# dmMaze/comic-text-detector

Hardware: AMD Instinct MI355X
Metric: pages/sec at 1024x1024 bs=32 (end-to-end detector, device-resident pages) (higher is better)
Workload: dtype f16

## Files before the change

### comic-text-detector_amd/csrc/kernels_twlds.hip

```cpp
#include <algorithm>

#include "kernels.h"
#include "tail.h"

namespace {

constexpr int TL_MAXT = 1024;

struct Geo {
  int W, H, wp, words;
  unsigned last;
};

__device__ __forceinline__ unsigned lds_ld(const unsigned* p) {
  return __hip_atomic_load(p, __ATOMIC_RELAXED, __HIP_MEMORY_SCOPE_WORKGROUP);
}
__device__ __forceinline__ void lds_st(unsigned* p, unsigned v) {
  __hip_atomic_store(p, v, __ATOMIC_RELAXED, __HIP_MEMORY_SCOPE_WORKGROUP);
}

struct Row3 {
  unsigned prev, cur, nxt;
};
__device__ __forceinline__ Row3 row3(const unsigned* p, const Geo& g, int y, int wi) {
  Row3 r{0u, 0u, 0u};
  if ((unsigned)y < (unsigned)g.H) {
    const unsigned* q = p + y * g.wp + wi;
    r.cur = q[0];
    if (wi > 0) r.prev = q[-1];
    if (wi + 1 < g.wp) r.nxt = q[1];
  }
  return r;
}
template <int K> __device__ __forceinline__ unsigned shk(const Row3& r) {
  if constexpr (K == 0) return r.cur;
  else if constexpr (K > 0) return (r.cur >> K) | (r.nxt << (32 - K));
  else return (r.cur << -K) | (r.prev >> (32 + K));
}
__device__ __forceinline__ unsigned ring3(const Row3& r) { return shk<-1>(r) | r.cur | shk<1>(r); }

__device__ __forceinline__ unsigned upto(int p) { return ~(~1u << p); }

__device__ __forceinline__ void load32(const uint8_t* p, int n, unsigned* v) {
  if (n >= 32) {
    __builtin_memcpy(v, p, 16);
    __builtin_memcpy(v + 4, p + 16, 16);
    return;
  }
#pragma unroll
  for (int j = 0; j < 8; ++j) {
    unsigned x = 0;
    if (4 * j + 4 <= n) {
      __builtin_memcpy(&x, p + 4 * j, 4);
    } else {
      for (int k = 0; k < 3; ++k)
        if (4 * j + k < n) x |= (unsigned)p[4 * j + k] << (8 * k);
    }
    v[j] = x;
  }
}

__device__ __forceinline__ unsigned gt60_nibble(unsigned x) {
  const unsigned t = (((x & 0x7f7f7f7fu) + 0x43434343u) | x) & 0x80808080u;
  const unsigned g = t >> 7;
  return (g | (g >> 7) | (g >> 14) | (g >> 21)) & 0xfu;
}

__device__ __forceinline__ int gray3(unsigned b, unsigned g, unsigned r) {
  return (int)((b * 3735u + g * 19235u + r * 9798u + 16384u) >> 15);
}

__device__ __forceinline__ unsigned uf_find(unsigned* parent, unsigned a) {
  for (;;) {
    const unsigned p = lds_ld(parent + a);
    if (p == a) return a;
    const unsigned gp = lds_ld(parent + p);
    if (gp != p) lds_st(parent + a, gp);
    a = gp;
  }
}
__device__ __forceinline__ void uf_union(unsigned* parent, unsigned a, unsigned b) {
  for (;;) {
    a = uf_find(parent, a);
    b = uf_find(parent, b);
    if (a == b) return;
    if (a < b) {
      const unsigned t = a;
      a = b;
      b = t;
    }
    if (atomicCAS(parent + a, a, b) == a) return;
  }
}

struct TLdsArgs {
  const TWin* wins;
  const TBand* bands;
  const int* order;
  int dilate;
  int max_words, rlay;
  int rcap;
  int* ovf;
};

__global__ __launch_bounds__(TL_MAXT) void tw_lds_kernel(TLdsArgs a) {
  extern __shared__ __attribute__((aligned(16))) unsigned lds[];
  const int t = threadIdx.x, lane = t & 63, wave = t >> 6;
  const int TL_NT = blockDim.x, NWV = TL_NT >> 6;
  const int widx = a.order[blockIdx.x];
  const TWin w = a.wins[widx];
  Geo g;
  g.W = w.w, g.H = w.h, g.wp = (w.w + 31) >> 5, g.words = g.wp * g.H;
  g.last = (w.w & 31) ? ((1u << (w.w & 31)) - 1u) : 0xffffffffu;
  const int MW = a.max_words, RL = a.rlay, RC = a.rcap;
  unsigned* const pred = lds;
  unsigned* const merged = lds + MW;
  unsigned* const cand = lds + 2 * MW;
  unsigned short* const base = (unsigned short*)(lds + 3 * MW);
  unsigned* const parent = lds + 3 * MW + ((MW + 1) >> 1);
  int* const acc = (int*)(parent + RL);
  unsigned* const red = parent + 2 * RL;
  unsigned* const tmp = parent;
  auto validw = [&](int wi) { return wi == g.wp - 1 ? g.last : 0xffffffffu; };
  const int y_t = t / g.wp, wi_t = t - y_t * g.wp;
  const int dy_t = TL_NT / g.wp, dwi_t = TL_NT - dy_t * g.wp;
  auto for_words = [&](auto&& fn) {
    int y = y_t, wi = wi_t;
    for (int i = t; i < g.words; i += TL_NT) {
      fn(i, y, wi);
      wi += dwi_t, y += dy_t;
      if (wi >= g.wp) wi -= g.wp, ++y;
    }
  };

  for_words([&](int i, int y, int wi) {
    unsigned v[8];
    load32(w.mask + (size_t)(w.y1 + y) * w.mask_w + w.x1 + 32 * wi, g.W - 32 * wi, v);
    unsigned bits = 0;
#pragma unroll
    for (int j = 0; j < 8; ++j) bits |= gt60_nibble(v[j]) << (4 * j);
    tmp[i] = bits & validw(wi);
    merged[i] = 0;
  });
  __syncthreads();
  for_words([&](int i, int y, int wi) {
    auto ext = [&](int yy, int ww) -> unsigned {
      if ((unsigned)yy >= (unsigned)g.H || (unsigned)ww >= (unsigned)g.wp) return 0xffffffffu;
      return tmp[yy * g.wp + ww] | ~validw(ww);
    };
    const unsigned cur = ext(y, wi), prev = ext(y, wi - 1), nxt = ext(y, wi + 1);
    pred[i] = cur & ((cur << 1) | (prev >> 31)) & ((cur >> 1) | (nxt << 31)) & ext(y - 1, wi) & ext(y + 1, wi) & validw(wi);
  });
  __syncthreads();

  const int seg = (g.words + TL_NT - 1) / TL_NT;
  auto starts_of = [&](int i, int wi) -> unsigned {
    const unsigned c = cand[i], cl = wi > 0 ? cand[i - 1] : 0u;
    return c & ~((c << 1) | (cl >> 31));
  };
  auto scan_runs = [&]() -> int {
    const int i0 = min(t * seg, g.words), i1 = min(i0 + seg, g.words);
    int cnt = 0;
    {
      int wi = i0 % g.wp;
      for (int i = i0; i < i1; ++i) {
        cnt += __popc(starts_of(i, wi));
        if (++wi == g.wp) wi = 0;
      }
    }
    int inc = cnt;
#pragma unroll
    for (int off = 1; off < 64; off <<= 1) {
      const int v = __shfl_up(inc, off);
      if (lane >= off) inc += v;
    }
    if (lane == 63) red[wave] = (unsigned)inc;
    __syncthreads();
    int before = inc - cnt;
    int total = 0;
    for (int k = 0; k < NWV; ++k) {
      const int v = (int)red[k];
      before += k < wave ? v : 0;
      total += v;
    }
    {
      int wi = i0 % g.wp, run = before;
      for (int i = i0; i < i1; ++i) {
        base[i] = (unsigned short)run;
        const int n = __popc(starts_of(i, wi));
        for (int k = run; k < run + n && k < RL; ++k) parent[k] = (unsigned)k, acc[k] = 0;
        run += n;
        if (++wi == g.wp) wi = 0;
      }
    }
    __syncthreads();
    return total;
  };
  auto rid_from = [](unsigned b, unsigned s, int p) -> unsigned { return b + (unsigned)__popc(s & upto(p)) - 1u; };
  auto for_groups = [&](unsigned v, auto&& fn) {
    while (v) {
      const unsigned lb = v & (0u - v);
      const unsigned grp = v & ~(v + lb);
      fn(__ffs((int)v) - 1, grp);
      v &= ~grp;
    }
  };
  auto link_and = [&](auto&& fn) {
    for_words([&](int i, int y, int wi) {
      const unsigned c = cand[i];
      if (!c) return;
      const unsigned cl = wi > 0 ? cand[i - 1] : 0u;
      const unsigned sc = c & ~((c << 1) | (cl >> 31)), bc = base[i];
      unsigned up = 0, ul = 0, ur = 0, su = 0, bu = 0;
      if (y > 0) {
        up = cand[i - g.wp];
        if (wi > 0) ul = cand[i - g.wp - 1];
        if (wi + 1 < g.wp) ur = cand[i - g.wp + 1];
        su = up & ~((up << 1) | (ul >> 31));
        bu = base[i - g.wp];
      }
      for_groups(c, [&](int p, unsigned grp) {
        const unsigned me = rid_from(bc, sc, p);
        fn(i, grp, me);
        if (y == 0) return;
        const unsigned an = up & (grp | (grp << 1) | (grp >> 1));
        unsigned reps = an & ~(an << 1);
        while (reps) {
          const int q = __ffs((int)reps) - 1;
          reps &= reps - 1;
          uf_union(parent, me, rid_from(bu, su, q));
        }
        if ((grp & 1u) && (ul >> 31)) uf_union(parent, me, bu - 1u);
        if ((grp >> 31) && (ur & 1u)) uf_union(parent, me, (unsigned)base[i - g.wp + 1] + ((up >> 31) ? 0u : 1u) - 1u);
      });
    });
  };
  auto fold_to_roots = [&](int n) {
    for (int i = t; i < n; i += TL_NT) {
      const unsigned r = uf_find(parent, (unsigned)i);
      if (r != (unsigned)i) {
        const int v = acc[i];
        if (v) atomicAdd(acc + r, v);
      }
    }
    __syncthreads();
  };
  auto or_accepted = [&]() {
    for_words([&](int i, int, int wi) {
      const unsigned c = cand[i];
      if (!c) return;
      const unsigned cl = wi > 0 ? cand[i - 1] : 0u;
      const unsigned sc = c & ~((c << 1) | (cl >> 31)), bc = base[i];
      unsigned add = 0;
      for_groups(c, [&](int p, unsigned grp) {
        if (acc[uf_find(parent, rid_from(bc, sc, p))] > 0) add |= grp;
      });
      if (add) merged[i] |= add;
    });
    __syncthreads();
  };
  bool overflow = false;

  for (int r = 0; r < w.nband && !overflow; ++r) {
    const TBand bd = a.bands[w.band0 + r];
    for_words([&](int i, int y, int wi) {
      const int npx = min(32, g.W - 32 * wi);
      const uint8_t* src = w.img + ((size_t)(w.y1 + y) * w.img_w + w.x1 + 32 * wi) * 3;
      unsigned v[24];
      load32(src, min(32, 3 * npx), v);
      load32(src + 32, min(32, max(0, 3 * npx - 32)), v + 8);
      load32(src + 64, min(32, max(0, 3 * npx - 64)), v + 16);
      unsigned bits = 0;
      auto byte_at = [&](int o) { return (v[o >> 2] >> (8 * (o & 3))) & 0xffu; };
      if (bd.kind == 0) {
#pragma unroll
        for (int k = 0; k < 32; ++k) {
          const int gr = gray3(byte_at(3 * k), byte_at(3 * k + 1), byte_at(3 * k + 2));
          bits |= ((gr >= bd.lo && gr <= bd.hi) ? 1u : 0u) << k;
        }
      } else {
        const int ch = bd.kind - 1;
#pragma unroll
        for (int k = 0; k < 32; ++k) {
          const unsigned c0 = byte_at(3 * k), c1 = byte_at(3 * k + 1), c2 = byte_at(3 * k + 2);
          bits |= (((int)(ch == 0 ? c0 : (ch == 1 ? c1 : c2)) > bd.lo) ? 1u : 0u) << k;
        }
      }
      if (bd.invert) bits = ~bits;
      tmp[i] = bits & validw(wi);
    });
    __syncthreads();
    for_words([&](int i, int y, int wi) {
      const Row3 c0 = row3(tmp, g, y, wi);
      unsigned out = c0.cur;
      if (out) {
        const Row3 m1 = row3(tmp, g, y - 1, wi), p1 = row3(tmp, g, y + 1, wi), m2 = row3(tmp, g, y - 2, wi), p2 = row3(tmp, g, y + 2, wi);
        const unsigned up = ring3(m1), dn = ring3(p1), cur = c0.cur;
        const unsigned single = cur & ~(shk<-1>(c0) | shk<1>(c0) | up | dn);
        const unsigned hl = cur & shk<1>(c0) & ~(shk<-1>(c0) | shk<2>(c0) | up | dn | shk<2>(m1) | shk<2>(p1));
        const unsigned hr = cur & shk<-1>(c0) & ~(shk<-2>(c0) | shk<1>(c0) | up | dn | shk<-2>(m1) | shk<-2>(p1));
        const unsigned vt = cur & p1.cur & ~(shk<-1>(c0) | shk<1>(c0) | shk<-1>(p1) | shk<1>(p1) | up | ring3(p2));
        const unsigned vb = cur & m1.cur & ~(shk<-1>(c0) | shk<1>(c0) | shk<-1>(m1) | shk<1>(m1) | dn | ring3(m2));
        out = cur & ~(single | hl | hr | vt | vb);
      }
      cand[i] = out;
    });
    __syncthreads();
    const int nr = scan_runs();
    if (nr > RC) {
      overflow = true;
      break;
    }
    link_and([&](int i, unsigned grp, unsigned me) {
      const unsigned nm = grp & ~merged[i];
      const int wgt = __popc(nm & pred[i]) - __popc(nm & ~pred[i]);
      if (wgt) atomicAdd(acc + me, wgt);
    });
    __syncthreads();
    fold_to_roots(nr);
    or_accepted();
  }

  if (!overflow) {
    if (a.dilate) {
      for_words([&](int i, int y, int wi) {
        unsigned v = 0;
#pragma unroll
        for (int dy = -1; dy <= 1; ++dy) {
          const Row3 r = row3(merged, g, y + dy, wi);
          v |= ring3(r);
        }
        tmp[i] = v & validw(wi);
      });
      __syncthreads();
    }
    unsigned cnt = 0;
    for_words([&](int i, int, int wi) {
      const unsigned m = a.dilate ? tmp[i] : merged[i];
      merged[i] = m;
      cand[i] = ~m & validw(wi);
      cnt += (unsigned)__popc(m);
    });
    for (int off = 32; off > 0; off >>= 1) cnt += __shfl_down(cnt, off);
    __syncthreads();
    if (lane == 0) red[wave] = cnt;
    if (t == 0) red[16] = 0u, red[17] = 0u, red[18] = 0u;
    __syncthreads();
    unsigned a0 = 0;
    for (int k = 0; k < NWV; ++k) a0 += red[k];
    __syncthreads();
    const int nr = scan_runs();
    if (nr > RC) {
      overflow = true;
    } else {
      link_and([&](int, unsigned grp, unsigned me) { atomicAdd(acc + me, __popc(grp)); });
      __syncthreads();
      fold_to_roots(nr);
      for (int i = t; i < nr + 1; i += TL_NT) {
        const bool is = i == nr || parent[i] == (unsigned)i;
        if (is) atomicMax(red + 16, (i == nr ? a0 : (unsigned)acc[i]) + 1u);
      }
      __syncthreads();
      const unsigned mx = red[16] - 1u;
      for (int i = t; i < nr + 1; i += TL_NT) {
        const bool is = i == nr || parent[i] == (unsigned)i;
        if (!is) continue;
        const unsigned ar = i == nr ? a0 : (unsigned)acc[i];
        if (ar == mx) atomicAdd(red + 17, 1u);
        else atomicMax(red + 18, ar + 1u);
      }
      __syncthreads();
      const long long thr = red[17] >= 2u ? (long long)mx : (long long)red[18] - 1;
      if (thr >= 0) {
        for (int i = t; i < nr; i += TL_NT)
          if (parent[i] == (unsigned)i) acc[i] = (long long)acc[i] < thr ? 0 : -(1 << 30);
        __syncthreads();
        for_words([&](int i, int, int wi) {
          const unsigned c = cand[i];
          if (!c) return;
          const unsigned cl = wi > 0 ? cand[i - 1] : 0u;
          const unsigned sc = c & ~((c << 1) | (cl >> 31)), bc = base[i];
          for_groups(c, [&](int p, unsigned grp) {
            const int wgt = __popc(grp & pred[i]) - __popc(grp & ~pred[i]);
            if (wgt) atomicAdd(acc + uf_find(parent, rid_from(bc, sc, p)), wgt);
          });
        });
        __syncthreads();
        or_accepted();
      }
    }
  }
  if (overflow) {
    if (t == 0) a.ovf[widx] = 1;
    return;
  }
  for_words([&](int i, int y, int wi) {
    const unsigned m = merged[i];
    if (!m) return;
    const size_t idx0 = (size_t)(w.y1 + y) * w.out_w + w.x1 + 32 * wi;
#pragma unroll
    for (int j = 0; j < 8; ++j) {
      const unsigned nib = (m >> (4 * j)) & 0xfu;
      if (!nib) continue;
      const unsigned v = ((nib & 1u) ? 0xffu : 0u) | ((nib & 2u) ? 0xff00u : 0u) | ((nib & 4u) ? 0xff0000u : 0u) |
                         ((nib & 8u) ? 0xff000000u : 0u);
      const size_t idx = idx0 + 4 * j;
      unsigned* ap = (unsigned*)(w.out + (idx & ~(size_t)3));
      const unsigned long long v2 = (unsigned long long)v << (8 * (idx & 3));
      if ((unsigned)v2) atomicOr(ap, (unsigned)v2);
      if ((unsigned)(v2 >> 32)) atomicOr(ap + 1, (unsigned)(v2 >> 32));
    }
  });
}

}

size_t tw_lds_bytes(int max_words, int rcap) {
  const int rlay = std::max(rcap, (max_words + 1) / 2);
  return ((size_t)3 * max_words + (max_words + 1) / 2 + (size_t)2 * rlay + 20) * 4;
}

int tw_lds_rcap(int max_words) { return std::min(65000, std::max(1024, (int)((long long)max_words * g_tw_lds_runs_x10 / 10))); }

bool launch_tw_lds(const TWin* wins, const TBand* bands, const int* order, int n, int max_words, int rcap, int dilate, int* ovf,
                   hipStream_t st, TwLdsLaunch* used) {
  if (n <= 0) return true;
  TLdsArgs a;
  a.wins = wins, a.bands = bands, a.order = order, a.dilate = dilate, a.max_words = max_words;
  a.rcap = std::min(rcap, 65000), a.rlay = std::max(a.rcap, (max_words + 1) / 2);
  a.ovf = ovf;
  const size_t bytes = tw_lds_bytes(max_words, a.rcap);
  const int nt = g_tw_lds_threads >= 1024 ? 1024 : (g_tw_lds_threads >= 512 ? 512 : 256);
  if (used) *used = TwLdsLaunch{n, max_words, a.rcap, nt, (int)bytes, 0};
  if (bytes > 48 * 1024 &&
      hipFuncSetAttribute((const void*)tw_lds_kernel, hipFuncAttributeMaxDynamicSharedMemorySize, (int)bytes) != hipSuccess) {
    (void)hipGetLastError();
    if (used) used->refused = 1;
    return false;
  }
  hipLaunchKernelGGL(tw_lds_kernel, dim3(n), dim3(nt), bytes, st, a);
  return true;
}
```

Measured before the change: 3337.

## Skip fruitless band rounds, vectorize band rendering, and exit early on empty windows

The band render loop now reads pixels with an aligned word load plus byte realignment, and it evaluates the gray or channel threshold with dot-product instructions and a single sign test instead of per-pixel branching. Band weights are now accumulated per run before linking. If no run in the block gets a positive weight, the link, fold and OR steps are skipped for that band. Windows with an empty merged mask return before the hole-filling stage, and union attempts a direct CAS first. Optional phase timing instrumentation is added behind a compile flag. The main risk is a change in semantics: weights are now attached to raw run ids before union, which relies on fold_to_roots aggregating them.

```diff
diff --git a/comic-text-detector_amd/csrc/kernels_twlds.hip b/comic-text-detector_amd/csrc/kernels_twlds.hip
--- a/comic-text-detector_amd/csrc/kernels_twlds.hip
+++ b/comic-text-detector_amd/csrc/kernels_twlds.hip
@@ -1,4 +1,5 @@
 #include <algorithm>
+#include <cstdio>
 
 #include "kernels.h"
 #include "tail.h"
@@ -41,33 +42,26 @@
 
 __device__ __forceinline__ unsigned upto(int p) { return ~(~1u << p); }
 
-__device__ __forceinline__ void load32(const uint8_t* p, int n, unsigned* v) {
-  if (n >= 32) {
-    __builtin_memcpy(v, p, 16);
-    __builtin_memcpy(v + 4, p + 16, 16);
+template <int NV> __device__ __forceinline__ void load_words(const uint8_t* p, int n, unsigned* v) {
+  if (n >= 4 * NV) {
+#pragma unroll
+    for (int j = 0; j < NV; j += 4) __builtin_memcpy(v + j, p + 4 * j, 16);
     return;
   }
-#pragma unroll
-  for (int j = 0; j < 8; ++j) {
-    unsigned x = 0;
-    if (4 * j + 4 <= n) {
-      __builtin_memcpy(&x, p + 4 * j, 4);
-    } else {
-      for (int k = 0; k < 3; ++k)
-        if (4 * j + k < n) x |= (unsigned)p[4 * j + k] << (8 * k);
-    }
-    v[j] = x;
-  }
+  const uintptr_t at = (uintptr_t)p;
+  const unsigned* q = (const unsigned*)(at & ~(uintptr_t)3);
+  const int off = (int)(at & 3), last = (off + n - 1) >> 2;
+  unsigned w[NV + 1];
+#pragma unroll
+  for (int k = 0; k <= NV; ++k) w[k] = q[min(k, last)];
+#pragma unroll
+  for (int j = 0; j < NV; ++j) v[j] = __builtin_amdgcn_alignbyte(w[j + 1], w[j], (unsigned)off);
 }
 
 __device__ __forceinline__ unsigned gt60_nibble(unsigned x) {
   const unsigned t = (((x & 0x7f7f7f7fu) + 0x43434343u) | x) & 0x80808080u;
   const unsigned g = t >> 7;
   return (g | (g >> 7) | (g >> 14) | (g >> 21)) & 0xfu;
-}
-
-__device__ __forceinline__ int gray3(unsigned b, unsigned g, unsigned r) {
-  return (int)((b * 3735u + g * 19235u + r * 9798u + 16384u) >> 15);
 }
 
 __device__ __forceinline__ unsigned uf_find(unsigned* parent, unsigned a) {
@@ -80,6 +74,7 @@
   }
 }
 __device__ __forceinline__ void uf_union(unsigned* parent, unsigned a, unsigned b) {
+  if (atomicCAS(parent + a, a, b) == a) return;
   for (;;) {
     a = uf_find(parent, a);
     b = uf_find(parent, b);
@@ -92,6 +87,30 @@
     if (atomicCAS(parent + a, a, b) == a) return;
   }
 }
+
+#ifdef CTD_MEASURE_KNOBS
+enum TwPhase {
+  PH_PRED, PH_RENDER, PH_FILTER, PH_SCAN, PH_WEIGH, PH_LINK, PH_FOLD, PH_OR, PH_EMPTY, PH_H_PREP, PH_H_SCAN, PH_H_LINK, PH_H_FOLD,
+  PH_H_REST, PH_COMMIT, PH_N
+};
+constexpr int TW_PHASE_EVERY = 400;
+__device__ unsigned long long g_tw_phase[PH_N + 4];
+#define TW_MARK(k)                                                                   \
+  do {                                                                               \
+    if (t == 0) {                                                                    \
+      const unsigned long long now_ = wall_clock64();                                \
+      atomicAdd(g_tw_phase + (k), now_ - mark_);                                     \
+      mark_ = now_;                                                                  \
+    }                                                                                \
+  } while (0)
+#define TW_COUNT(k)                                                                  \
+  do {                                                                               \
+    if (t == 0) atomicAdd(g_tw_phase + PH_N + (k), 1ull);                            \
+  } while (0)
+#else
+#define TW_MARK(k) ((void)0)
+#define TW_COUNT(k) ((void)0)
+#endif
 
 struct TLdsArgs {
   const TWin* wins;
@@ -108,6 +127,10 @@
   const int t = threadIdx.x, lane = t & 63, wave = t >> 6;
   const int TL_NT = blockDim.x, NWV = TL_NT >> 6;
   const int widx = a.order[blockIdx.x];
+#ifdef CTD_MEASURE_KNOBS
+  unsigned long long mark_ = wall_clock64();
+  TW_COUNT(0);
+#endif
   const TWin w = a.wins[widx];
   Geo g;
   g.W = w.w, g.H = w.h, g.wp = (w.w + 31) >> 5, g.words = g.wp * g.H;
@@ -122,6 +145,12 @@
   unsigned* const red = parent + 2 * RL;
   unsigned* const tmp = parent;
   auto validw = [&](int wi) { return wi == g.wp - 1 ? g.last : 0xffffffffu; };
+  if (t == 0) red[19] = 0u;
+  auto block_any = [&](bool mine, unsigned gen) -> bool {
+    if (mine) red[19] = gen;
+    __syncthreads();
+    return red[19] == gen;
+  };
   const int y_t = t / g.wp, wi_t = t - y_t * g.wp;
   const int dy_t = TL_NT / g.wp, dwi_t = TL_NT - dy_t * g.wp;
   auto for_words = [&](auto&& fn) {
@@ -135,7 +164,7 @@
 
   for_words([&](int i, int y, int wi) {
     unsigned v[8];
-    load32(w.mask + (size_t)(w.y1 + y) * w.mask_w + w.x1 + 32 * wi, g.W - 32 * wi, v);
+    load_words<8>(w.mask + (size_t)(w.y1 + y) * w.mask_w + w.x1 + 32 * wi, min(32, g.W - 32 * wi), v);
     unsigned bits = 0;
 #pragma unroll
     for (int j = 0; j < 8; ++j) bits |= gt60_nibble(v[j]) << (4 * j);
@@ -152,6 +181,7 @@
     pred[i] = cur & ((cur << 1) | (prev >> 31)) & ((cur >> 1) | (nxt << 31)) & ext(y - 1, wi) & ext(y + 1, wi) & validw(wi);
   });
   __syncthreads();
+  TW_MARK(PH_PRED);
 
   const int seg = (g.words + TL_NT - 1) / TL_NT;
   auto starts_of = [&](int i, int wi) -> unsigned {
@@ -263,33 +293,36 @@
 
   for (int r = 0; r < w.nband && !overflow; ++r) {
     const TBand bd = a.bands[w.band0 + r];
+    int A, C;
+    unsigned coef_lo, coef_hi;
+    if (bd.kind == 0) {
+      const int lo = max(bd.lo, 0), hi = min(bd.hi, 255);
+      A = lo * 32768 - 16384, C = hi * 32768 + 16383 - A;
+      coef_lo = 151u | (35u << 8) | (70u << 16), coef_hi = 14u | (75u << 8) | (38u << 16);
+    } else {
+      A = min(max(bd.lo, -1), 255) + 1, C = 255 - A;
+      coef_lo = 1u << (8 * (bd.kind - 1)), coef_hi = 0u;
+    }
     for_words([&](int i, int y, int wi) {
       const int npx = min(32, g.W - 32 * wi);
       const uint8_t* src = w.img + ((size_t)(w.y1 + y) * w.img_w + w.x1 + 32 * wi) * 3;
       unsigned v[24];
-      load32(src, min(32, 3 * npx), v);
-      load32(src + 32, min(32, max(0, 3 * npx - 32)), v + 8);
-      load32(src + 64, min(32, max(0, 3 * npx - 64)), v + 16);
-      unsigned bits = 0;
-      auto byte_at = [&](int o) { return (v[o >> 2] >> (8 * (o & 3))) & 0xffu; };
-      if (bd.kind == 0) {
-#pragma unroll
-        for (int k = 0; k < 32; ++k) {
-          const int gr = gray3(byte_at(3 * k), byte_at(3 * k + 1), byte_at(3 * k + 2));
-          bits |= ((gr >= bd.lo && gr <= bd.hi) ? 1u : 0u) << k;
-        }
-      } else {
-        const int ch = bd.kind - 1;
-#pragma unroll
-        for (int k = 0; k < 32; ++k) {
-          const unsigned c0 = byte_at(3 * k), c1 = byte_at(3 * k + 1), c2 = byte_at(3 * k + 2);
-          bits |= (((int)(ch == 0 ? c0 : (ch == 1 ? c1 : c2)) > bd.lo) ? 1u : 0u) << k;
-        }
-      }
+      load_words<24>(src, 3 * npx, v);
+      unsigned outside = 0;
+#pragma unroll
+      for (int k = 31; k >= 0; --k) {
+        const int j = (3 * k) >> 2, sh = (3 * k) & 3;
+        const unsigned px = sh == 0 ? v[j] : __builtin_amdgcn_alignbyte(j + 1 < 24 ? v[j + 1] : 0u, v[j], sh);
+        const int d1 = (int)((__builtin_amdgcn_udot4(px, coef_hi, 0u, false) << 8) + __builtin_amdgcn_udot4(px, coef_lo, (unsigned)-A, false));
+        outside = __builtin_amdgcn_alignbit(outside, (unsigned)(d1 | (C - d1)), 31);
+      }
+      unsigned bits = ~outside;
       if (bd.invert) bits = ~bits;
       tmp[i] = bits & validw(wi);
     });
     __syncthreads();
+    TW_MARK(PH_RENDER);
+    TW_COUNT(2);
     for_words([&](int i, int y, int wi) {
       const Row3 c0 = row3(tmp, g, y, wi);
       unsigned out = c0.cur;
@@ -306,19 +339,51 @@
       cand[i] = out;
     });
     __syncthreads();
+    TW_MARK(PH_FILTER);
     const int nr = scan_runs();
+    TW_MARK(PH_SCAN);
     if (nr > RC) {
       overflow = true;
       break;
     }
-    link_and([&](int i, unsigned grp, unsigned me) {
-      const unsigned nm = grp & ~merged[i];
-      const int wgt = __popc(nm & pred[i]) - __popc(nm & ~pred[i]);
-      if (wgt) atomicAdd(acc + me, wgt);
+    bool positive = false;
+    for_words([&](int i, int, int wi) {
+      const unsigned c = cand[i];
+      if (!c) return;
+      const unsigned cl = wi > 0 ? cand[i - 1] : 0u;
+      const unsigned sc = c & ~((c << 1) | (cl >> 31)), bc = base[i];
+      const unsigned open = ~merged[i], pr = pred[i];
+      for_groups(c, [&](int p, unsigned grp) {
+        const unsigned nm = grp & open;
+        const int wgt = __popc(nm & pr) - __popc(nm & ~pr);
+        if (wgt) atomicAdd(acc + rid_from(bc, sc, p), wgt);
+        positive |= wgt > 0;
+      });
     });
-    __syncthreads();
+    const bool fruitful = block_any(positive, (unsigned)r + 1u);
+    TW_MARK(PH_WEIGH);
+    if (!fruitful) {
+      TW_COUNT(3);
+      continue;
+    }
+    link_and([](int, unsigned, unsigned) {});
+    __syncthreads();
+    TW_MARK(PH_LINK);
     fold_to_roots(nr);
+    TW_MARK(PH_FOLD);
     or_accepted();
+    TW_MARK(PH_OR);
+  }
+
+  if (!overflow && g.H <= RC) {
+    unsigned any = 0;
+    for_words([&](int i, int, int) { any |= merged[i]; });
+    const bool empty = !block_any(any != 0u, (unsigned)w.nband + 1u);
+    TW_MARK(PH_EMPTY);
+    if (empty) {
+      TW_COUNT(1);
+      return;
+    }
   }
 
   if (!overflow) {
@@ -349,13 +414,17 @@
     unsigned a0 = 0;
     for (int k = 0; k < NWV; ++k) a0 += red[k];
     __syncthreads();
+    TW_MARK(PH_H_PREP);
     const int nr = scan_runs();
+    TW_MARK(PH_H_SCAN);
     if (nr > RC) {
       overflow = true;
     } else {
       link_and([&](int, unsigned grp, unsigned me) { atomicAdd(acc + me, __popc(grp)); });
       __syncthreads();
+      TW_MARK(PH_H_LINK);
       fold_to_roots(nr);
+      TW_MARK(PH_H_FOLD);
       for (int i = t; i < nr + 1; i += TL_NT) {
         const bool is = i == nr || parent[i] == (unsigned)i;
         if (is) atomicMax(red + 16, (i == nr ? a0 : (unsigned)acc[i]) + 1u);
@@ -388,6 +457,7 @@
         __syncthreads();
         or_accepted();
       }
+      TW_MARK(PH_H_REST);
     }
   }
   if (overflow) {
@@ -411,6 +481,7 @@
       if ((unsigned)(v2 >> 32)) atomicOr(ap + 1, (unsigned)(v2 >> 32));
     }
   });
+  TW_MARK(PH_COMMIT);
 }
 
 }
@@ -439,5 +510,20 @@
     return false;
   }
   hipLaunchKernelGGL(tw_lds_kernel, dim3(n), dim3(nt), bytes, st, a);
+#ifdef CTD_MEASURE_KNOBS
+  static int launches = 0;
+  if (++launches % TW_PHASE_EVERY == 0) {
+    unsigned long long h[PH_N + 4];
+    if (hipMemcpyFromSymbol(h, HIP_SYMBOL(g_tw_phase), sizeof h) == hipSuccess) {
+      static const char* const names[PH_N] = {"prediction", "render", "filter", "scan_runs", "weigh", "link_and", "fold_to_roots",
+                                              "or_accepted", "empty_test", "holes_prep", "holes_scan", "holes_link", "holes_fold",
+                                              "holes_rest", "commit"};
+      fprintf(stderr, "twlds phases after %d launches: blocks %llu empty_exits %llu rounds %llu rounds_skipped %llu |", launches,
+              h[PH_N], h[PH_N + 1], h[PH_N + 2], h[PH_N + 3]);
+      for (int k = 0; k < PH_N; ++k) fprintf(stderr, " %s %llu", names[k], h[k]);
+      fprintf(stderr, " (ticks of 10 ns, summed over blocks)\n");
+    }
+  }
+#endif
   return true;
 }
```

Result: slower. 3260 (-2.3%).
